# bcgsc/ntJoin

Hardware: AMD Instinct MI355X
Metric: Gbp/s minimizer-sketch+graph-build (k=32,w=1000) (higher is better)
Workload: dtype u64

## Files before the change

### ntjoin_amd/csrc/sketch.hip

```cpp
#include <algorithm>
#include <chrono>
#include <cmath>
#include <cstdlib>
#include <cstring>
#include <functional>
#include <type_traits>

#include "mxg_internal.h"
#include "nthash_dev.h"
#include "scan_kernels.h"
#include "sketch_bs.h"

namespace mxg {

enum Scratch {
    SC_CAND_H, SC_CAND_K, SC_CAND_C, SC_SEL, SC_BSUM, SC_CTRL, SC_ARENA, SC_STRIP_CNT, SC_STRIP_META,
    SC_GAPS, SC_WAVE_CNT, SC_ST_HASH, SC_ST_POS, SC_ST_REC, SC_ST_FWD, SC_G_HASH, SC_G_POS,
    SC_G_REC, SC_G_FWD, SC_V_RUNS, SC_V_STRIP0, SC_V_G0, SC_V_NK, SC_V_REC, SC_V_RUN0, SC_V_DROP, SC_CNT256, SC_WAVE_TOT,
    SC_GR_HASH, SC_GR_POS, SC_GR_REC, SC_GR_CNT, SC_GR_KEY, SC_GD_HASH, SC_GD_POS, SC_GD_REC,
    SC_CS_H, SC_CS_K, SC_CS_C,
    SC_GB_WORK,
    SC_COUNT
};
static_assert(SC_COUNT <= 40, "scratch pool too small");
// ... 2262 lines not shown
        if (rc != MXG_OK) return rc;
        return ev_end();
    }

    BsSelGeom sel_geom(const Assembly *a, const BatchGeom &g, double frac) const
    {
        return bs_select_geom(a->S_sparse, a->sel_H, h->cfg.w, frac, g.n_strips, (uint32_t)env_u64(h, "MXG_SEL_QCAP", 0), (uint32_t)env_u64(h, "MXG_SEL_RK", 0));
    }
    bool ctrl_cleared = false;
    int clear_sel_ctrl(const BsSelGeom &b)
    {
        int rc;
        if ((rc = flush_emit(nullptr)) != MXG_OK) return rc;
        const size_t ctrl_bytes = ((size_t)CTRL_WORDS + sup_words(b.n_slices) + 2 * 64 * 32) * 4;
        MXG_HIP(h, sc(SC_CTRL).ensure(ctrl_bytes));
        MXG_HIP(h, hipMemsetAsync(sc(SC_CTRL).p, 0, ctrl_bytes, st));
        ctrl_cleared = true;
        return MXG_OK;
    }
    int enqueue_sel(Assembly *a, const Tables &T, const BatchGeom &g, const BsSelGeom &b, uint32_t tau_hi, OutArrays &out,
                    uint32_t *ctrl_host, const ChainIO *io)
    {
        int rc;
        if ((rc = flush_emit(nullptr)) != MXG_OK) return rc;
        MXG_HIP(h, sc(SC_GAPS).ensure((size_t)GAP_CAP * 16));
        n_wave_sup = 0;
        const size_t ctrl_bytes = ((size_t)CTRL_WORDS + sup_words(b.n_slices) + 2 * 64 * 32) * 4;
        MXG_HIP(h, sc(SC_CTRL).ensure(ctrl_bytes));
        MXG_HIP(h, sc(SC_CNT256).ensure((size_t)b.n_slices * 4 + 64));
        const size_t n_ent = (size_t)b.n_slices * b.rk;
        MXG_HIP(h, sc(SC_CS_H).ensure(n_ent * 16));
        const size_t ovf_ent = (size_t)b.n_ovf * (b.ovf_cap + 2 * SEL_PAD);
        MXG_HIP(h, sc(SC_CAND_H).ensure(ovf_ent * 8));
        MXG_HIP(h, sc(SC_CAND_K).ensure(ovf_ent * 4));
        if (!ctrl_cleared) MXG_HIP(h, hipMemsetAsync(sc(SC_CTRL).p, 0, ctrl_bytes, st));
        ctrl_cleared = false;
        if ((rc = ev_begin(0, false, 2)) != MXG_OK) return rc;
        BsSelParams bp{};
        bp.bm = a->d_bs_out.as<uint32_t>() + 4;
        bp.packed = a->d_packed;
        bp.runx = a->d_runx.as<RunX>();
        bp.strip_run = T.d_strip_run;
        bp.ctg_drop = T.d_ctg_drop;
        bp.ptab = h->d_init_tab.as<uint4>() + 256;
        bp.n_strips_asm = (*T.strip0_sparse)[T.runs->size()];
        bp.strip_lo = g.strip_lo;
        bp.strip_hi = g.strip_hi;
        bp.S = a->S_sparse;
        bp.H = b.H;
        bp.T = b.T;
        bp.n_slices = b.n_slices;
        bp.w = h->cfg.w;
        bp.tau = (uint64_t)tau_hi << 32;
        bp.qcap = b.qcap;
        bp.ovf_h = sc(SC_CAND_H).as<uint64_t>();
        bp.ovf_e = sc(SC_CAND_K).as<uint32_t>();
        bp.ovf_cap = b.ovf_cap;
        bp.n_ovf = b.n_ovf;
        bp.ovf_next = sc(SC_CTRL).as<uint32_t>() + 12;
        bp.rk = b.rk;
        bp.cs = sc(SC_CS_H).as<uint4>();
        bp.cnt = sc(SC_CNT256).as<uint32_t>();
        bp.sup = sel_sup(0);
        bp.gaps = sc(SC_GAPS).as<uint4>();
        bp.gap_cap = GAP_CAP - SEL_IREQ_CAP;
        bp.ireq = sc(SC_GAPS).as<uint4>() + bp.gap_cap;
        bp.ireq_cap = SEL_IREQ_CAP - 8u;
        bp.gap_nmax = (io && io->dev_gaps && h->cfg.w <= ST_WMAX && !knob_set(h, "MXG_STRETCH_DENSE") && !knob_set(h, "MXG_GAP_WHOLE")) ? GAP_DEV_NMAX : 0u;
        bp.ctrl = sc(SC_CTRL).as<uint32_t>();
        bp.cand_spread = sel_sup(0) + sup_words(b.n_slices);
        bp.ablate = (uint32_t)env_u64(h, "MXG_SEL_ABLATE", 0);
        bp.inl_amax = knob_u64(h, "MXG_SEL_INLINE", 1) && b.n_slices < (1u << 24) ? bs_select_inline_amax(h->cfg.w) : 0u;
        if ((rc = launch_bs_select(h, bp, b, st)) != MXG_OK) return rc;
        const bool late = knob_u64(h, "MXG_STAGGER", 1) == 2;
        if (h->ev_sel_done[slot] && !late) MXG_HIP(h, hipEventRecord(h->ev_sel_done[slot], st));
        h->stat_sel_slices += b.n_slices;
        const bool dev = io && io->dev_gaps;
        if (timing && !fine) {
            if ((rc = ev_end()) != MXG_OK || (rc = ev_begin(0, false, 1)) != MXG_OK) return rc;
        }
        if ((rc = ev_next(3)) != MXG_OK) return rc;
        if (bp.inl_amax) {
            SelStretchParams sp{};
            sp.packed = bp.packed;
            sp.runs = T.d_runs;
            sp.ctg_run0 = T.d_ctg_run0;
            sp.ctg_drop = T.d_ctg_drop;
            sp.byte_tab = h->d_init_tab.as<uint4>();
            sp.tab = h->tab;
            sp.w = bp.w;
            sp.amax = bp.inl_amax;
            sp.rk = bp.rk;
            sp.cs = bp.cs;
            sp.cnt = bp.cnt;
            sp.sup = bp.sup;
            sp.ireq = bp.ireq;
            sp.ireq_cap = bp.ireq_cap;
            sp.ctrl = bp.ctrl;
            sp.tickets = bp.cand_spread + 64 * 32;
            sp.ablate = (uint32_t)env_u64(h, "MXG_SST_ABLATE", 0);
            sp.gaps = bp.gaps;
            sp.gap_cap = bp.gap_cap;
            sp.gap_nmax = bp.gap_nmax;
            if ((rc = launch_sel_stretch(h, sp, st)) != MXG_OK) return rc;
        }
        if (dev && (rc = enqueue_dev_gaps(a, T, ctrl_host)) != MXG_OK) return rc;
        if (defer_emit && io && !io->wait && !io->base_in && !io->base_out) {
            if ((rc = ev_end()) != MXG_OK) return rc;
            const Tables *Tp = &T;
            DevBuf *oh = out.hash, *op = out.pos, *orc = out.rec, *of = out.fwd;
            const uint64_t on = out.n;
            const ChainIO ioc = *io;
            const uint32_t rk = b.rk, gc = gcap, np = n_place;
            uint32_t *const no = n_out;
            const uint32_t *cs = bp.cand_spread;
            pending_emit = [=](hipEvent_t behind) -> int {
                int rc2;
                if (behind) MXG_HIP(h, hipStreamWaitEvent(st, behind, 0));
                if ((rc2 = ev_begin(0, false, fine ? 4 : 1)) != MXG_OK) return rc2;
                const uint32_t gc0 = gcap, np0 = n_place;
                uint32_t *const no0 = n_out;
                gcap = gc; n_place = np; n_out = no;
                rc2 = emit(a->d_packed, *Tp, (uint32_t)n_ent, *oh, *op, *orc, *of, on, true, ctrl_host, &ioc, rk, (uint32_t)n_ent, cs);
                gcap = gc0; n_place = np0; n_out = no0;
                if (rc2 != MXG_OK) return rc2;
                return ev_end();
            };
            return MXG_OK;
        }
        if ((rc = ev_next(4)) != MXG_OK) return rc;
        if (io && io->wait) MXG_HIP(h, hipStreamWaitEvent(st, io->wait, 0));
        rc = emit(a->d_packed, T, (uint32_t)n_ent, *out.hash, *out.pos, *out.rec, *out.fwd, out.n, true, ctrl_host, io, b.rk,
                  (uint32_t)n_ent, bp.cand_spread);
        if (rc != MXG_OK) return rc;
        if (h->ev_sel_done[slot] && late) MXG_HIP(h, hipEventRecord(h->ev_sel_done[slot], st));
        return ev_end();
    }
    std::function<int(hipEvent_t)> pending_emit;
    bool defer_emit = false;
    int flush_emit(hipEvent_t behind)
    {
        if (!pending_emit) return MXG_OK;
        auto f = std::move(pending_emit);
        pending_emit = nullptr;
        return f(behind);
    }

    int complete_batch(Assembly *a, const Tables &T, const BatchGeom &g, OutArrays &out, const uint32_t *ctrl, uint32_t n_cap)
    {
        const size_t c0 = g.c0, c1 = g.c1;
// ... 1359 lines not shown
```

### ntjoin_amd/csrc/sketch_bs.h

```cpp
#pragma once
#include "mxg_internal.h"

namespace mxg {

#ifndef MXG_BS_CHUNK_DEFINED
#define MXG_BS_CHUNK_DEFINED
constexpr uint32_t BS_CHUNK = 65536;
#endif

constexpr uint32_t SEL_PAD = 8;
constexpr uint32_t SEL_REQ = 8;
constexpr uint32_t SEL_GAP_DROP = 0x80000000u;
constexpr uint32_t SEL_MAX_H = 12;
constexpr uint32_t SEL_INL_R = 4;
constexpr uint32_t SEL_INL_PIECES = 6;
constexpr uint32_t SEL_INL_TMP = 128;
constexpr uint32_t SEL_IREQ_CAP = 1u << 18;

struct BsSelParams {
    const uint32_t *bm;
    const uint32_t *packed;
    const RunX *runx;
    const uint32_t *strip_run;
    const uint8_t *ctg_drop;
    const uint4 *ptab;
    uint32_t n_strips_asm;
    uint32_t strip_lo, strip_hi;
    uint32_t S, H, T;
    uint32_t n_slices;
    uint32_t w;
    uint64_t tau;
    uint32_t qcap;
    uint64_t *ovf_h;
    uint32_t *ovf_e;
    uint32_t ovf_cap, n_ovf;
    uint32_t *ovf_next;
    uint32_t rk;
    uint4 *cs;
    uint32_t *cnt, *sup;
    uint4 *gaps;
    uint32_t gap_cap;
    uint32_t gap_nmax;
    uint32_t *cand_spread;
    uint32_t *ctrl;
    uint32_t ablate;
    uint32_t inl_amax;
    uint4 *ireq;
    uint32_t ireq_cap;
};

struct SelStretchParams {
    const uint32_t *packed;
    const Run *runs;
    const uint32_t *ctg_run0;
    const uint8_t *ctg_drop;
    const uint4 *byte_tab;
    HashTab tab;
    uint32_t w, amax, rk;
    uint4 *cs;
    uint32_t *cnt, *sup;
    const uint4 *ireq;
    uint32_t ireq_cap;
    uint32_t *ctrl;
    uint32_t *tickets;
    uint4 *gaps;
    uint32_t gap_cap, gap_nmax;
    uint32_t ablate;
};
uint32_t bs_select_inline_amax(uint32_t w);
int launch_sel_stretch(mxg_handle *h, const SelStretchParams &p, hipStream_t st);

struct BsSelGeom {
    uint32_t H, T, n_slices, rk, qcap, waves, ovf_cap, n_ovf;
    size_t lds;
    bool ok;
};
uint32_t bs_select_halo(const Assembly *a, uint32_t S, uint32_t w);
BsSelGeom bs_select_geom(uint32_t S, uint32_t H, uint32_t w, double frac, uint32_t n_strips, uint32_t qcap_force, uint32_t rk_force = 0);
int launch_bs_select(mxg_handle *h, const BsSelParams &p, const BsSelGeom &g, hipStream_t st);

bool bs_possible(const mxg_handle *h, const Assembly *a);
int bs_prepare(mxg_handle *h, Assembly *a);
int bs_edges(mxg_handle *h, Assembly *a, hipStream_t st);
int bs_hash(mxg_handle *h, Assembly *a, uint32_t tau_hi, hipStream_t st);

}
```

### ntjoin_amd/csrc/sketch_bs.hip

```cpp
#include <algorithm>
#include <cmath>
#include <mutex>

#include "bs_kernels.h"
#include "nthash_dev.h"
#include "scan_kernels.h"
#include "sketch_bs.h"

namespace mxg {

namespace {

struct __attribute__((packed, aligned(4))) Words3 {
    uint32_t w0, w1, w2;
};
struct __attribute__((packed, aligned(4))) Words4 {
    uint32_t w0, w1, w2, w3;
};
template <int B>
__device__ __forceinline__ uint32_t byte_x16(const uint32_t x)
{
    uint32_t r;
#if defined(__HIP_DEVICE_COMPILE__)
    static_assert(B >= 0 && B < 4, "byte of a word");
// ... 48 lines not shown
__device__ __forceinline__ uint32_t sel_bits(const uint32_t w_lo, const uint32_t w_hi, const uint32_t sh, const uint32_t len, const uint32_t j)
{
    const uint32_t bits = __builtin_amdgcn_alignbit(w_hi, w_lo, sh);
    const uint32_t k0 = 32u * j;
    const uint32_t nvalid = len > k0 ? min(len - k0, 32u) : 0u;
    return bits & (nvalid >= 32u ? 0xFFFFFFFFu : ((1u << nvalid) - 1u));
}

struct StripRegs {
    uint64_t b;
    uint32_t len, cg, k0, nk;
};
__device__ __forceinline__ StripRegs strip_of(const BsSelParams &p, const bool in, const uint32_t sS, const uint32_t ri)
{
    StripRegs r;
    r.b = 0; r.len = 0; r.cg = 0xFFFFFFFFu; r.k0 = 0; r.nk = 0;
    if (in) {
        const RunX run = p.runx[ri];
        const uint32_t j0 = sS - run.strip0S;
        r.len = min(p.S, run.n_kmers - j0);
        r.b = run.base_off + j0;
        r.cg = run.contig;
        r.k0 = run.kidx0 + j0;
        r.nk = run.nk;
    }
    return r;
}
__device__ __forceinline__ StripRegs strip_from_run(const BsSelParams &p, const bool in, const uint32_t sS, const RunX &run)
{
    const uint32_t j0 = sS - run.strip0S;
    StripRegs r;
    r.len = in ? min(p.S, run.n_kmers - j0) : 0u;
    r.b = in ? run.base_off + j0 : 0ull;
    r.cg = in ? run.contig : 0xFFFFFFFFu;
    r.k0 = in ? run.kidx0 + j0 : 0u;
    r.nk = in ? run.nk : 0u;
    return r;
}
__device__ __forceinline__ StripRegs load_strip(const BsSelParams &p, const int64_t s64)
{
    const bool in = s64 >= 0 && s64 < (int64_t)p.n_strips_asm;
    const uint32_t s = in ? (uint32_t)s64 : 0u;
    return strip_of(p, in, s * p.S, in ? p.strip_run[s] : 0u);
}

__device__ __forceinline__ uint32_t wave_inclusive_dpp(uint32_t v)
{
    v += (uint32_t)__builtin_amdgcn_update_dpp(0, (int)v, 0x111, 0xf, 0xf, false);
    v += (uint32_t)__builtin_amdgcn_update_dpp(0, (int)v, 0x112, 0xf, 0xf, false);
    v += (uint32_t)__builtin_amdgcn_update_dpp(0, (int)v, 0x114, 0xf, 0xf, false);
    v += (uint32_t)__builtin_amdgcn_update_dpp(0, (int)v, 0x118, 0xf, 0xf, false);
    v += (uint32_t)__builtin_amdgcn_update_dpp(0, (int)v, 0x142, 0xa, 0xf, false);
    v += (uint32_t)__builtin_amdgcn_update_dpp(0, (int)v, 0x143, 0xc, 0xf, false);
    return v;
}

__device__ __forceinline__ const BsSelParams *sel_rare_params()
{
#if defined(__HIP_DEVICE_COMPILE__)
    const void *q = (const void *)__builtin_amdgcn_kernarg_segment_ptr();
    asm volatile("" : "+s"(q));
    return static_cast<const BsSelParams *>(q);
#else
    return nullptr;
#endif
}
__device__ __forceinline__ void push_gap(uint4 *gaps, uint32_t gap_cap, uint32_t *ctrl, uint32_t nmax, uint32_t w, uint32_t c, uint32_t lo,
                                         uint32_t hi, uint32_t hint)
{
    uint32_t s = lo, flag = 0u;
    for (;;) {
        const uint32_t e = nmax && hi - s >= nmax ? s + nmax - 1u : hi;
        const uint32_t idx = atomicAdd(&ctrl[1], 1u);
        if (idx < gap_cap) gaps[idx] = make_uint4(c, s, e, hint | flag);
        if (e == hi) break;
        s = e - w + 1u;
        flag = SEL_GAP_DROP;
    }
}
__device__ __forceinline__ void sel_push_gap(const BsSelParams &, uint32_t c, uint32_t lo, uint32_t hi, uint32_t hint)
{
    const BsSelParams *q = sel_rare_params();
    push_gap(q->gaps, q->gap_cap, q->ctrl, q->gap_nmax, q->w, c, lo, hi, hint);
}

__device__ __forceinline__ uint32_t stretch_end(const BsSelParams &p, const uint4 *ptab, const uint32_t lane, int64_t s_next, const uint32_t c,
                                                const uint32_t nk)
{
    const uint32_t nwords = (p.S + 31u) / 32u;
    for (;; s_next += 64) {
        const StripRegs r = load_strip(p, s_next + lane);
        const bool stop = r.cg != c;
        uint32_t kfound = 0xFFFFFFFFu;
        if (!stop) {
            const uint32_t *bw = p.bm + (r.b >> 5);
            const uint32_t sh = (uint32_t)r.b & 31u;
            uint32_t w0 = bw[0];
            for (uint32_t j = 0; j < nwords && kfound == 0xFFFFFFFFu; ++j) {
                const uint32_t w1 = bw[j + 1u];
                uint32_t bits = sel_bits(w0, w1, sh, r.len, j);
                w0 = w1;
                for (; bits; bits &= bits - 1u) {
                    const uint32_t ju = 32u * j + (uint32_t)__builtin_ctz(bits);
                    if (hash32_pos(p.packed, r.b + ju, ptab) < p.tau) {
                        kfound = r.k0 + ju;
                        break;
                    }
                }
            }
        }
        const uint64_t mf = __ballot(kfound != 0xFFFFFFFFu), ms = __ballot(stop);
        const uint64_t ev = mf | ms;
        if (ev) {
            const int first = __builtin_ctzll(ev);
            if ((mf >> first) & 1ull) return (uint32_t)__builtin_amdgcn_readlane((int)kfound, first) - 1u;
            return nk - 1u;
        }
    }
}

constexpr uint32_t SEL_SI = 6;

__host__ __device__ inline uint32_t sel_wave_lds(uint32_t qcap)
{
    return (qcap + 2u * SEL_PAD) * 12u + SEL_SI * 64u * 4u + SEL_REQ * 16u + SEL_REQ * 16u + 16u;
}

struct SelCtx {
    const uint4 *ptab;
    uint32_t *si;
    uint4 *req;
    uint32_t *misc;
    uint32_t lane, sl, own_end;
    bool has_drop;
    int64_t s_first;
    uint32_t nreal, own_lo, own_hi;
};

template <bool GLOB>
__device__ __forceinline__ void sel_sync()
{
    if (GLOB) __threadfence_block();
    else __builtin_amdgcn_wave_barrier();
}

template <int NB, bool GLOB>
__device__ __forceinline__ void sel_collect(const BsSelParams &p, SelCtx &c, uint64_t *lh, uint32_t *le, const uint32_t cap,
                                            const uint32_t (&bt)[NB], const uint32_t at0, const uint32_t tot)
{
    const uint32_t lane = c.lane, H = p.H;
    const uint32_t qn = min(tot, cap);
    {
        uint32_t at = at0;
#pragma unroll
        for (uint32_t j = 0; j < (uint32_t)NB; ++j) {
            uint32_t bits = bt[j];
            const uint32_t item0 = lane | ((32u * j) << 6);
            for (; bits; bits &= bits - 1u, ++at) le[at] = item0 + ((uint32_t)__builtin_ctz(bits) << 6);
        }
    }
    const uint32_t *s_blo = c.si, *s_bhi = c.si + 64, *s_f = c.si + 320;
    sel_sync<GLOB>();
    c.nreal = c.own_lo = c.own_hi = 0;
    if (p.ablate == 2) return;
    uint32_t nreal = 0, own_lo = 0, own_hi = 0;
    constexpr uint32_t NR = 4;
    for (uint32_t q0 = 0; q0 < qn; q0 += 64u * NR) {
        uint32_t item[NR];
        Words3 wv[NR];
        uint32_t shv[NR];
#pragma unroll
        for (uint32_t r = 0; r < NR; ++r) {
            const uint32_t q = q0 + 64u * r + lane;
            const bool act = q < qn;
            item[r] = act ? le[q] : 0u;
            const uint32_t l2 = item[r] & 63u;
            const uint64_t b = (((uint64_t)s_bhi[l2] << 32) | s_blo[l2]) + (item[r] >> 6);
            wv[r] = Words3{0u, 0u, 0u};
            if (act) wv[r] = *reinterpret_cast<const Words3 *>(p.packed + (b >> 4));
            shv[r] = ((uint32_t)b & 15u) * 2u;
        }
#pragma unroll
        for (uint32_t r = 0; r < NR; ++r) {
            if (q0 + 64u * r >= qn) break;
            const bool act = q0 + 64u * r + lane < qn;
            const uint32_t l2 = item[r] & 63u, ju = item[r] >> 6;
            const uint64_t h = act ? hash32_words(wv[r].w0, wv[r].w1, wv[r].w2, shv[r], c.ptab) : ~0ull;
            const bool real = act && h < p.tau;
            const uint64_t m = __ballot(real);
            const uint32_t rank = __builtin_amdgcn_mbcnt_hi((uint32_t)(m >> 32), __builtin_amdgcn_mbcnt_lo((uint32_t)m, 0u));
            if (real) {
                le[nreal + rank] = ((s_f[l2] + ju) << 6) | l2;
                lh[nreal + rank] = h;
            }
            own_lo += (uint32_t)__popcll(__ballot(real && l2 < H));
            own_hi += (uint32_t)__popcll(__ballot(real && l2 < c.own_end));
            nreal += (uint32_t)__popcll(m);
        }
    }
    if (lane < SEL_PAD) {
        le[-1 - (int)lane] = 0u;
        lh[-1 - (int)lane] = ~0ull;
        le[nreal + lane] = 0xFFFFFFFFu;
        lh[nreal + lane] = ~0ull;
    }
    sel_sync<GLOB>();
    c.nreal = nreal; c.own_lo = own_lo; c.own_hi = own_hi;
}

template <bool GLOB>
__device__ __forceinline__ void sel_decide(const BsSelParams &p, SelCtx &c, const uint64_t *lh, const uint32_t *le, const StripRegs &sr,
                                           const uint32_t f, bool &flag)
{
    const uint32_t lane = c.lane, sl = c.sl, H = p.H, w = p.w, wm1 = w - 1u, nreal = c.nreal;
    const bool has_drop = c.has_drop;
    const uint32_t lim = 64u * wm1 + 63u;
    const uint32_t *s_c = c.si + 128, *s_k0 = c.si + 192, *s_nk = c.si + 256, *s_f = c.si + 320;
    const uint32_t cov_c = (uint32_t)__builtin_amdgcn_readlane((int)sr.cg, 63);
    const uint32_t cov_kend = (uint32_t)__builtin_amdgcn_readlane((int)(sr.k0 + sr.len), 63);
    const uint32_t cov_nk = (uint32_t)__builtin_amdgcn_readlane((int)sr.nk, 63);
    const bool cov_open = cov_c != 0xFFFFFFFFu && cov_kend < cov_nk;
    auto push_req = [&](uint32_t cg, uint32_t lo, uint32_t hi) {
        const uint32_t q = atomicAdd(&c.misc[2], 1u);
        if (q < SEL_REQ) reinterpret_cast<uint4 *>(c.misc + 4)[q] = make_uint4(cg, lo, hi, 0u);
        else sel_push_gap(p, cg, lo, hi, sl * p.rk);
    };
    auto report = [&](uint32_t cg, uint32_t k_from, uint32_t nk, uint32_t nx) {
        bool same = false;
        uint32_t k2 = 0;
        if (nx < nreal) {
            const uint32_t e2 = le[nx], l2 = e2 & 63u;
            same = s_c[l2] == cg;
            k2 = s_k0[l2] + ((e2 >> 6) - s_f[l2]);
        }
        if (same) {
            if (k2 - k_from >= w) push_req(cg, k_from, k2 - 1u);
        } else if (nk - k_from >= w) {
            if (!(cov_open && cg == cov_c)) {
                push_req(cg, k_from, nk - 1u);
            } else {
                const uint32_t at = atomicAdd(&c.misc[0], 1u);
                if (at < SEL_REQ) c.req[at] = make_uint4(cg, k_from, nk, 0u);
            }
        }
    };
    uint32_t n_sel = 0;
    for (uint32_t i0 = c.own_lo; i0 < c.own_hi; i0 += 64u) {
        const bool live = i0 + lane < c.own_hi;
        const uint32_t i = live ? i0 + lane : i0;
        const uint32_t e = le[i], l1 = e & 63u;
        const uint64_t h = lh[i];
        const uint32_t kx = s_k0[l1] + ((e >> 6) - s_f[l1]), cg = s_c[l1], nk = s_nk[l1];
        const uint32_t e_lo = e - lim;
        uint32_t al = 0u;
        bool ldone = !live;
        for (uint32_t t = 1; !ldone; t += SEL_PAD) {
            uint32_t ae[SEL_PAD];
            uint64_t ah[SEL_PAD];
#pragma unroll
            for (uint32_t u = 0; u < SEL_PAD; ++u) {
// ... 23 lines not shown
            const uint32_t c0 = bh[0] <= h ? be[0] : n, c1 = bh[1] <= h ? be[1] : n, c2 = bh[2] <= h ? be[2] : n, c3 = bh[3] <= h ? be[3] : n;
            const uint32_t c4 = bh[4] <= h ? be[4] : n, c5 = bh[5] <= h ? be[5] : n, c6 = bh[6] <= h ? be[6] : n, c7 = bh[7] <= h ? be[7] : n;
            const uint32_t bl = min(min(min(c0, c1), c2), min(min(min(c3, c4), c5), min(c6, c7)));
            const bool blocked = bl <= e_hi;
            s = blocked ? false : s;
            rdone = blocked || be[SEL_PAD - 1] > e_hi;
        }
        if (has_drop && s && kx <= wm1 && L == kx && sel_rare_params()->ctg_drop[cg]) s = false;
        const uint64_t bm = __ballot(s);
        if (s) {
            const uint32_t dst = n_sel + __builtin_amdgcn_mbcnt_hi((uint32_t)(bm >> 32), __builtin_amdgcn_mbcnt_lo((uint32_t)bm, 0u));
            if (dst < p.rk) p.cs[(size_t)sl * p.rk + dst] = make_uint4((uint32_t)h, (uint32_t)(h >> 32), kx, cg);
        }
        n_sel += (uint32_t)__popcll(bm);
        if (live && le[i + 1u] - e >= 64u * (w + 1u)) report(cg, kx + 1u, nk, i + 1u);
    }
    if (lane >= H && lane < c.own_end && sr.len && sr.k0 == 0) {
        uint32_t lo = 0, hi = nreal;
        while (lo < hi) {
            const uint32_t mid = (lo + hi) >> 1;
            if ((le[mid] >> 6) < f) lo = mid + 1u; else hi = mid;
        }
        report(sr.cg, 0u, sr.nk, lo);
    }
    sel_sync<GLOB>();
    if (lane == 0) {
        if (n_sel > p.rk) flag = true;
        count_publish(p.cnt, p.sup, sl, min(n_sel, p.rk));
    }
    const uint32_t n_req = c.misc[0];
    if (n_req) {
        if (n_req > SEL_REQ) flag = true;
        for (uint32_t r = 0; r < min(n_req, SEL_REQ); ++r) {
            const uint4 rq = c.req[r];
            const uint32_t k_end = stretch_end(p, c.ptab, lane, c.s_first + 64, rq.x, rq.z);
            if (lane == 0 && k_end + 1u - rq.y >= w) push_req(rq.x, rq.y, k_end);
        }
        sel_sync<GLOB>();
        if (lane == 0) c.misc[0] = 0;
    }
    if (__builtin_expect(c.misc[2] != 0u, 0)) {
        const BsSelParams *pr = sel_rare_params();
        const uint32_t n_i = min(c.misc[2], SEL_REQ);
        const bool to_kernel = pr->inl_amax != 0u;
        uint32_t base = 0xFFFFFFFFu - SEL_REQ;
        if (to_kernel && lane == 0) base = atomicAdd(&pr->ctrl[15], n_i);
        base = (uint32_t)__builtin_amdgcn_readfirstlane((int)base);
        uint32_t ln = lane;
#if defined(__HIP_DEVICE_COMPILE__)
        asm volatile("" : "+v"(ln));
#endif
        if (ln < n_i) {
            const uint32_t *g = c.misc + 4u + 4u * ln;
            if (base + n_i <= pr->ireq_cap) pr->ireq[base + ln] = make_uint4(g[0], g[1], g[2], sl | (ln << 24) | (n_i << 27));
            else sel_push_gap(p, g[0], g[1], g[2], sl * pr->rk);
        }
        __builtin_amdgcn_wave_barrier();
        if (lane == 0) c.misc[2] = 0;
    }
}

}

template <int NWC, int NWX>
__global__ __launch_bounds__(1024) void k_bs_select(const BsSelParams p)
{
    static_assert(NWC % 4 == 0, "the strips' bitmap words are requested four at a time");
    static_assert(NWX < NWC, "one word more than the strip's bits is read (the bits are shifted into place)");
    constexpr int NB = NWX ? NWX : NWC - 1;
    extern __shared__ uint4 sel_lds[];
    uint4 *ptab = sel_lds;
    if ((uint32_t)(uintptr_t)sel_lds != 0u) __builtin_trap();
    for (uint32_t i = threadIdx.x; i < 2048u; i += blockDim.x) ptab[i] = p.ptab[i];
    const uint32_t lane = threadIdx.x & 63u, wib = threadIdx.x >> 6, nwv = blockDim.x >> 6;
    unsigned char *wb = reinterpret_cast<unsigned char *>(sel_lds + 2048) + (size_t)wib * sel_wave_lds(p.qcap);
    uint64_t *lh = reinterpret_cast<uint64_t *>(wb);
    uint32_t *le = reinterpret_cast<uint32_t *>(lh + p.qcap + 2u * SEL_PAD);
    SelCtx c;
    c.ptab = ptab;
    c.si = le + p.qcap + 2u * SEL_PAD;
    c.req = reinterpret_cast<uint4 *>(c.si + SEL_SI * 64u);
    c.misc = reinterpret_cast<uint32_t *>(c.req + SEL_REQ);
    c.lane = lane;
    c.has_drop = p.ctg_drop != nullptr;
    c.nreal = c.own_lo = c.own_hi = 0;
    uint32_t *blk_ticket = reinterpret_cast<uint32_t *>(reinterpret_cast<unsigned char *>(sel_lds + 2048) + (size_t)nwv * sel_wave_lds(p.qcap));
    if (threadIdx.x == 0) *blk_ticket = nwv;
    if (lane == 0) {
        c.misc[0] = 0;
        c.misc[2] = 0;
        c.misc[1] = 0xFFFFFFFFu;
    }
    __syncthreads();
    const uint32_t S = p.S, H = p.H, T = p.T, w = p.w;
    const uint32_t nwords = NWX ? (uint32_t)NWX : (S + 31u) / 32u;
    const uint32_t stride = gridDim.x * nwv, laneS = lane * S;
    uint32_t own_cands = 0;
    bool flag = false;
    auto slice_of = [&](uint32_t t) { return (t / nwv) * stride + blockIdx.x * nwv + (t % nwv); };
    uint32_t sl = slice_of(wib);
    const uint32_t sl_end = p.n_slices;
    auto first_strip = [&](uint32_t q) { return (int64_t)(p.strip_lo + q * T) - (int64_t)H; };
    StripRegs sr = sl < sl_end ? load_strip(p, first_strip(sl) + lane) : StripRegs{0, 0, 0xFFFFFFFFu, 0, 0};
    while (sl < sl_end) {
        uint32_t tk = 0;
        if (lane == 0) tk = atomicAdd(blk_ticket, 1u);
        const uint32_t sl_n = slice_of((uint32_t)__builtin_amdgcn_readfirstlane((int)tk));
        const uint32_t s_own0 = p.strip_lo + sl * T;
        c.sl = sl;
        c.s_first = first_strip(sl);
        c.own_end = H + min(T, p.strip_hi - s_own0);
        const uint32_t sn32 = p.strip_lo + sl_n * T - H + lane;
        const bool in_n = sl_n < sl_end && sn32 < p.n_strips_asm;
        const uint32_t s_n = in_n ? sn32 : 0u;
        const uint32_t ri_n = p.strip_run[s_n];
        const uint32_t sS_n = (sn32 - lane) * S + laneS;
        uint32_t wd[NWC];
        {
            const Words4 *bw = reinterpret_cast<const Words4 *>(p.bm + (sr.b >> 5));
#pragma unroll
            for (uint32_t u = 0; u < (uint32_t)NWC / 4u; ++u) {
                Words4 v{0u, 0u, 0u, 0u};
                if (sr.len && 4u * u <= nwords) v = bw[u];
                wd[4 * u] = v.w0; wd[4 * u + 1] = v.w1; wd[4 * u + 2] = v.w2; wd[4 * u + 3] = v.w3;
            }
        }
        const uint32_t len_p = (uint32_t)__builtin_amdgcn_update_dpp(0, (int)sr.len, 0x138, 0xf, 0xf, false);
        const uint32_t cg_p = (uint32_t)__builtin_amdgcn_update_dpp(-1, (int)sr.cg, 0x138, 0xf, 0xf, false);
        const uint32_t f = wave_inclusive_dpp(lane ? len_p + (sr.cg != cg_p ? w : 0u) : 2u * w);
        c.si[lane] = (uint32_t)sr.b;
        c.si[64u + lane] = (uint32_t)(sr.b >> 32);
        c.si[128u + lane] = sr.cg;
        c.si[192u + lane] = sr.k0;
        c.si[256u + lane] = sr.nk;
        c.si[320u + lane] = f;
        uint32_t bt[NB];
        uint32_t cnt = 0;
        {
            const uint32_t sh = (uint32_t)sr.b & 31u;
            const bool whole = (NWX || (S & 31u) == 0) && __ballot(sr.len != 0 && sr.len != S) == 0;
            if (whole) {
#pragma unroll
                for (uint32_t j = 0; j < (uint32_t)NB; ++j) bt[j] = j < nwords ? __builtin_amdgcn_alignbit(wd[j + 1], wd[j], sh) : 0u;
            } else {
#pragma unroll
                for (uint32_t j = 0; j < (uint32_t)NB; ++j) bt[j] = j < nwords ? sel_bits(wd[j], wd[j + 1], sh, sr.len, j) : 0u;
            }
#pragma unroll
            for (uint32_t j = 0; j < (uint32_t)NB; ++j) cnt += (uint32_t)__popc(bt[j]);
        }
        const uint32_t incl = wave_inclusive_dpp(cnt);
        const uint32_t tot = (uint32_t)__builtin_amdgcn_readlane((int)incl, 63);
        const RunX run_n = p.runx[ri_n];
        if (p.ablate == 1) {
            if (lane == 0) count_publish(p.cnt, p.sup, sl, 0u);
            own_cands += tot != 0;
        } else if (tot <= p.qcap) {
            sel_collect<NB, false>(p, c, lh + SEL_PAD, le + SEL_PAD, p.qcap, bt, incl - cnt, tot);
            if (p.ablate == 2 || p.ablate == 3) {
                if (lane == 0) count_publish(p.cnt, p.sup, sl, 0u);
                own_cands += 1u;
            } else {
                sel_decide<false>(p, c, lh + SEL_PAD, le + SEL_PAD, sr, f, flag);
            }
        } else {
            const BsSelParams *q = sel_rare_params();
            if (lane == 0 && c.misc[1] == 0xFFFFFFFFu) c.misc[1] = atomicAdd(q->ovf_next, 1u);
            __builtin_amdgcn_wave_barrier();
            const uint32_t region = c.misc[1];
            if (region < q->n_ovf) {
                const uint32_t ocap = q->ovf_cap;
                const size_t o = (size_t)region * (ocap + 2u * SEL_PAD) + SEL_PAD;
                sel_collect<NB, true>(p, c, q->ovf_h + o, q->ovf_e + o, ocap, bt, incl - cnt, tot);
                sel_decide<true>(p, c, q->ovf_h + o, q->ovf_e + o, sr, f, flag);
            } else {
                flag = true;
                c.own_lo = c.own_hi = 0;
                if (lane == 0) count_publish(p.cnt, p.sup, sl, 0u);
            }
        }
        own_cands += c.own_hi - c.own_lo;
        __builtin_amdgcn_wave_barrier();
        sr = strip_from_run(p, in_n, sS_n, run_n);
        sl = sl_n;
    }
    const uint32_t own_w = own_cands;
    if (lane == 0) {
        const BsSelParams *q = sel_rare_params();
        if (own_w) atomicAdd(&q->cand_spread[((blockIdx.x * nwv + wib) & 63u) * 32u], own_w);
        if (flag) q->ctrl[6] = q->ctrl[13] = 1;
    }
}

namespace {

struct InlBest {
    uint64_t h;
    uint32_t id;
};
template <int CTRL, int ROWS>
__device__ __forceinline__ InlBest inl_dpp(const InlBest v)
{
    InlBest o;
    const uint32_t lo = (uint32_t)__builtin_amdgcn_update_dpp(-1, (int)(uint32_t)v.h, CTRL, ROWS, 0xf, false);
    const uint32_t hi = (uint32_t)__builtin_amdgcn_update_dpp(-1, (int)(uint32_t)(v.h >> 32), CTRL, ROWS, 0xf, false);
    o.h = ((uint64_t)hi << 32) | lo;
    o.id = (uint32_t)__builtin_amdgcn_update_dpp(-1, (int)v.id, CTRL, ROWS, 0xf, false);
    return o;
}
template <bool OWN_LEFT>
__device__ __forceinline__ InlBest inl_scan(InlBest v)
{
#define MXG_INL_STEP(CTRL, ROWS)                                                   \
    {                                                                              \
        const InlBest g = inl_dpp<CTRL, ROWS>(v);                                  \
        const bool take = OWN_LEFT ? (g.id != 0xFFFFFFFFu && !(v.h < g.h)) : (g.h < v.h); \
        if (take) v = g;                                                           \
    }
    MXG_INL_STEP(0x111, 0xf)
    MXG_INL_STEP(0x112, 0xf)
    MXG_INL_STEP(0x114, 0xf)
    MXG_INL_STEP(0x118, 0xf)
    MXG_INL_STEP(0x142, 0xa)
    MXG_INL_STEP(0x143, 0xc)
#undef MXG_INL_STEP
    return v;
}
__device__ __forceinline__ InlBest inl_lane(const InlBest v, const int src_lane)
{
    InlBest o;
    o.h = __shfl(v.h, src_lane);
    o.id = __shfl(v.id, src_lane);
    return o;
}
// ... 120 lines not shown
        for (uint32_t r = 1; r < SEL_INL_R; ++r)
            if (r < R) last = ids[r];
        uint32_t prev = (uint32_t)__shfl((int)last, (int)lane - 1);
        if (lane == 0) prev = 0xFFFFFFFFu;
        uint32_t cnt = 0;
        bool em[SEL_INL_R];
#pragma unroll
        for (uint32_t r = 0; r < SEL_INL_R; ++r) {
            const uint32_t j = lane * R + r;
            em[r] = r < R && j <= a && ids[r] != prev && hs[r] != ~0ull && !(j == 0u && (lo != 0u || drop0));
            if (r < R && j <= a) prev = ids[r];
            cnt += em[r] ? 1u : 0u;
        }
        const uint32_t incl = wave_inclusive_dpp(cnt);
        const uint32_t tot = (uint32_t)__builtin_amdgcn_readlane((int)incl, 63);
        if (m + tot > cap_t) return 0xFFFFFFFFu;
        uint32_t at = m + incl - cnt;
#pragma unroll
        for (uint32_t r = 0; r < SEL_INL_R; ++r)
            if (em[r]) tmp[at++] = make_uint4((uint32_t)hs[r], (uint32_t)(hs[r] >> 32), k_from + lo + ids[r], cg);
        m += tot;
        __builtin_amdgcn_wave_barrier();
        if (lo + a >= a_tot) break;
        lo += a;
    }
    return m;
}

}

constexpr uint32_t SST_WAVES = 4;
__global__ __launch_bounds__(SST_WAVES * 64, 5) void k_sel_stretch(const SelStretchParams p)
{
    __shared__ uint4 byte_tab[256];
    __shared__ uint4 rtab[16];
    __shared__ uint64_t Xs[SST_WAVES][2 * 64 * SEL_INL_R];
    __shared__ uint4 tmps[SST_WAVES][SEL_INL_TMP];
    const uint32_t n_req = min(p.ctrl[15], p.ireq_cap);
    if (blockIdx.x * SST_WAVES >= n_req) return;
    for (uint32_t i = threadIdx.x; i < 256u; i += blockDim.x) byte_tab[i] = p.byte_tab[i];
    if (threadIdx.x < 16u) rtab[threadIdx.x] = p.tab.e[threadIdx.x];
    __syncthreads();
    const uint32_t lane = threadIdx.x & 63u, wv = threadIdx.x >> 6;
    uint64_t *X = Xs[wv];
    uint4 *tmp = tmps[wv];
    uint32_t *const ticket = p.tickets + ((blockIdx.x * SST_WAVES + wv) & 63u) * 32u;
    for (;;) {
        uint32_t r = 0;
        if (lane == 0) r = atomicAdd(ticket, 1u);
        r = (uint32_t)__builtin_amdgcn_readfirstlane((int)r) * 64u + ((blockIdx.x * SST_WAVES + wv) & 63u);
        if (r >= n_req) break;
        const uint4 mine = p.ireq[r + (lane & 7u)];
        const uint32_t w0 = (uint32_t)__builtin_amdgcn_readfirstlane((int)mine.w);
        if ((w0 >> 24) & 7u) continue;
        if (p.ablate & 8u) continue;
        const uint32_t n_i = min(w0 >> 27, SEL_REQ), sl = w0 & 0xFFFFFFu;
        const bool has = lane < n_i;
        const uint64_t my_key = has ? (((uint64_t)mine.x << 32) | mine.y) + 1ull : 0ull;
        uint4 *row = p.cs + (size_t)sl * p.rk;
        uint32_t n_cur = p.cnt[sl];
        uint64_t my_b = 0;
        bool my_ok = false;
        if (has) {
            uint32_t lo = p.ctg_run0[mine.x], hi = p.ctg_run0[mine.x + 1u];
            while (hi - lo > 1u) {
                const uint32_t mid = (lo + hi) >> 1;
                if (p.runs[mid].kidx0 <= mine.y) lo = mid; else hi = mid;
            }
            const Run run = p.runs[lo];
            my_ok = mine.z < run.kidx0 + run.n_kmers && mine.z - mine.y + 1u >= p.w && mine.z - mine.y + 1u - p.w <= p.amax * SEL_INL_PIECES;
            my_b = run.base_off + (mine.y - run.kidx0);
        }
        n_cur = (uint32_t)__builtin_amdgcn_readfirstlane((int)n_cur);
        uint4 e0 = make_uint4(0u, 0u, 0xFFFFFFFFu, 0xFFFFFFFFu), e1 = e0;
        if (lane < n_cur) e0 = row[lane];
        if (lane + 64u < n_cur) e1 = row[lane + 64u];
        const bool in_regs = n_cur <= 128u && n_i == 1u;
        uint32_t added = 0;
        uint64_t left = my_key;
        for (uint32_t it = 0; it < n_i; ++it) {
            uint64_t best = left;
#pragma unroll
            for (uint32_t d = 1; d < 8u; d <<= 1) {
                const uint64_t o = __shfl_xor(best, (int)d);
                best = o > best ? o : best;
            }
            best = __shfl(best, 0);
            const uint64_t holder = __ballot(left == best && best != 0ull);
            const int src = __builtin_ctzll(holder);
            if ((int)lane == src) left = 0ull;
            const uint32_t cg = (uint32_t)__shfl((int)mine.x, src), k_from = (uint32_t)__shfl((int)mine.y, src), k_to = (uint32_t)__shfl((int)mine.z, src);
            const uint64_t b_from = __shfl(my_b, src);
            const bool ok = __shfl((int)my_ok, src) != 0;
            const bool drop0 = k_from == 0u && p.ctg_drop && p.ctg_drop[cg];
            const uint64_t key = ((uint64_t)cg << 32) | k_from;
            uint32_t below = ((((uint64_t)e0.w << 32) | e0.z) < key ? 1u : 0u) + ((((uint64_t)e1.w << 32) | e1.z) < key ? 1u : 0u);
            for (uint32_t e = lane + 128u; e < n_cur - added; e += 64u) {
                const uint4 q = row[e];
                below += ((((uint64_t)q.w << 32) | q.z) < key) ? 1u : 0u;
            }
            uint32_t m = ok ? stretch_sketch(p, byte_tab, rtab, X, tmp, SEL_INL_TMP, cg, k_from, k_to, b_from, drop0) : 0xFFFFFFFFu;
            if (m != 0xFFFFFFFFu && n_cur + m > p.rk) m = 0xFFFFFFFFu;
            if (m == 0xFFFFFFFFu) {
                if (lane == 0) push_gap(p.gaps, p.gap_cap, p.ctrl, p.gap_nmax, p.w, cg, k_from, k_to, sl * p.rk);
                continue;
            }
            if (m == 0 || (p.ablate & 32u)) continue;
            const uint32_t at = wave_sum_u32(below);
            if (in_regs) {
// ... 204 lines not shown
```

Before: 2472.

## Prune dominated high-hash candidates before minimizer selection using low-hash coverage

Adds a lower hash threshold tau_lo (a fraction of tau, tunable through MXG_SEL_PRUNE) and, inside sel_collect, runs two wave-wide DPP max/min scans over the collected candidates. Candidates above tau_lo that sit between low-hash candidates spaced no more than w apart can never be window minimizers, so they are compacted away before sel_decide, and own counts are recomputed. This is meant to cut the work in the decide phase and in later stretch processing, at the cost of two extra passes over the candidate list and extra wave barriers. It also makes inline requests that overflow the request buffer write tombstones so the stretch kernel skips them, and adds a slice bounds check there.

```diff
diff --git a/ntjoin_amd/csrc/sketch.hip b/ntjoin_amd/csrc/sketch.hip
--- a/ntjoin_amd/csrc/sketch.hip
+++ b/ntjoin_amd/csrc/sketch.hip
@@ -2338,6 +2338,8 @@
         bp.n_slices = b.n_slices;
         bp.w = h->cfg.w;
         bp.tau = (uint64_t)tau_hi << 32;
+        const uint64_t prune = std::min<uint64_t>(env_u64(h, "MXG_SEL_PRUNE", 9), 23);
+        bp.tau_lo = tau_hi <= 0x80000000u ? (uint64_t)(((unsigned __int128)bp.tau * prune) / 24u) : 0ull;
         bp.qcap = b.qcap;
         bp.ovf_h = sc(SC_CAND_H).as<uint64_t>();
         bp.ovf_e = sc(SC_CAND_K).as<uint32_t>();
@@ -2352,6 +2354,7 @@
         bp.gap_cap = GAP_CAP - SEL_IREQ_CAP;
         bp.ireq = sc(SC_GAPS).as<uint4>() + bp.gap_cap;
         bp.ireq_cap = SEL_IREQ_CAP - 8u;
+        if (const uint64_t ic = env_u64(h, "MXG_SEL_IREQ_CAP", 0)) bp.ireq_cap = (uint32_t)std::min<uint64_t>(ic, bp.ireq_cap);
         bp.gap_nmax = (io && io->dev_gaps && h->cfg.w <= ST_WMAX && !knob_set(h, "MXG_STRETCH_DENSE") && !knob_set(h, "MXG_GAP_WHOLE")) ? GAP_DEV_NMAX : 0u;
         bp.ctrl = sc(SC_CTRL).as<uint32_t>();
         bp.cand_spread = sel_sup(0) + sup_words(b.n_slices);
@@ -2382,6 +2385,7 @@
             sp.sup = bp.sup;
             sp.ireq = bp.ireq;
             sp.ireq_cap = bp.ireq_cap;
+            sp.n_slices = bp.n_slices;
             sp.ctrl = bp.ctrl;
             sp.tickets = bp.cand_spread + 64 * 32;
             sp.ablate = (uint32_t)env_u64(h, "MXG_SST_ABLATE", 0);
diff --git a/ntjoin_amd/csrc/sketch_bs.h b/ntjoin_amd/csrc/sketch_bs.h
--- a/ntjoin_amd/csrc/sketch_bs.h
+++ b/ntjoin_amd/csrc/sketch_bs.h
@@ -16,6 +16,7 @@
 constexpr uint32_t SEL_INL_PIECES = 6;
 constexpr uint32_t SEL_INL_TMP = 128;
 constexpr uint32_t SEL_IREQ_CAP = 1u << 18;
+constexpr uint32_t SEL_IREQ_TOMB = 0xFFFFFFFFu;
 
 struct BsSelParams {
     const uint32_t *bm;
@@ -30,6 +31,7 @@
     uint32_t n_slices;
     uint32_t w;
     uint64_t tau;
+    uint64_t tau_lo;
     uint32_t qcap;
     uint64_t *ovf_h;
     uint32_t *ovf_e;
@@ -61,6 +63,7 @@
     uint32_t *cnt, *sup;
     const uint4 *ireq;
     uint32_t ireq_cap;
+    uint32_t n_slices;
     uint32_t *ctrl;
     uint32_t *tickets;
     uint4 *gaps;
diff --git a/ntjoin_amd/csrc/sketch_bs.hip b/ntjoin_amd/csrc/sketch_bs.hip
--- a/ntjoin_amd/csrc/sketch_bs.hip
+++ b/ntjoin_amd/csrc/sketch_bs.hip
@@ -124,6 +124,26 @@
     v += (uint32_t)__builtin_amdgcn_update_dpp(0, (int)v, 0x118, 0xf, 0xf, false);
     v += (uint32_t)__builtin_amdgcn_update_dpp(0, (int)v, 0x142, 0xa, 0xf, false);
     v += (uint32_t)__builtin_amdgcn_update_dpp(0, (int)v, 0x143, 0xc, 0xf, false);
+    return v;
+}
+__device__ __forceinline__ uint32_t wave_inclusive_max_dpp(uint32_t v)
+{
+    v = max(v, (uint32_t)__builtin_amdgcn_update_dpp(0, (int)v, 0x111, 0xf, 0xf, false));
+    v = max(v, (uint32_t)__builtin_amdgcn_update_dpp(0, (int)v, 0x112, 0xf, 0xf, false));
+    v = max(v, (uint32_t)__builtin_amdgcn_update_dpp(0, (int)v, 0x114, 0xf, 0xf, false));
+    v = max(v, (uint32_t)__builtin_amdgcn_update_dpp(0, (int)v, 0x118, 0xf, 0xf, false));
+    v = max(v, (uint32_t)__builtin_amdgcn_update_dpp(0, (int)v, 0x142, 0xa, 0xf, false));
+    v = max(v, (uint32_t)__builtin_amdgcn_update_dpp(0, (int)v, 0x143, 0xc, 0xf, false));
+    return v;
+}
+__device__ __forceinline__ uint32_t wave_inclusive_min_dpp(uint32_t v)
+{
+    v = min(v, (uint32_t)__builtin_amdgcn_update_dpp(-1, (int)v, 0x111, 0xf, 0xf, false));
+    v = min(v, (uint32_t)__builtin_amdgcn_update_dpp(-1, (int)v, 0x112, 0xf, 0xf, false));
+    v = min(v, (uint32_t)__builtin_amdgcn_update_dpp(-1, (int)v, 0x114, 0xf, 0xf, false));
+    v = min(v, (uint32_t)__builtin_amdgcn_update_dpp(-1, (int)v, 0x118, 0xf, 0xf, false));
+    v = min(v, (uint32_t)__builtin_amdgcn_update_dpp(-1, (int)v, 0x142, 0xa, 0xf, false));
+    v = min(v, (uint32_t)__builtin_amdgcn_update_dpp(-1, (int)v, 0x143, 0xc, 0xf, false));
     return v;
 }
 
@@ -207,6 +227,8 @@
     bool has_drop;
     int64_t s_first;
     uint32_t nreal, own_lo, own_hi;
+    uint32_t off;
+    uint32_t n_own;
 };
 
 template <bool GLOB>
@@ -215,6 +237,8 @@
     if (GLOB) __threadfence_block();
     else __builtin_amdgcn_wave_barrier();
 }
+
+constexpr uint64_t SEL_SHORT = 1ull << 63;
 
 template <int NB, bool GLOB>
 __device__ __forceinline__ void sel_collect(const BsSelParams &p, SelCtx &c, uint64_t *lh, uint32_t *le, const uint32_t cap,
@@ -233,8 +257,10 @@
     }
     const uint32_t *s_blo = c.si, *s_bhi = c.si + 64, *s_f = c.si + 320;
     sel_sync<GLOB>();
-    c.nreal = c.own_lo = c.own_hi = 0;
+    c.nreal = c.own_lo = c.own_hi = c.off = c.n_own = 0;
     if (p.ablate == 2) return;
+    const uint64_t tau_lo = p.tau_lo;
+    const uint32_t w = p.w;
     uint32_t nreal = 0, own_lo = 0, own_hi = 0;
     constexpr uint32_t NR = 4;
     for (uint32_t q0 = 0; q0 < qn; q0 += 64u * NR) {
@@ -270,6 +296,54 @@
             nreal += (uint32_t)__popcll(m);
         }
     }
+    c.n_own = own_hi - own_lo;
+    uint32_t off = 0;
+    if (tau_lo && p.ablate != 4) {
+        sel_sync<GLOB>();
+        uint32_t low_carry = 0;
+        for (uint32_t i0 = 0; i0 < nreal; i0 += 64u) {
+            const bool act = i0 + lane < nreal;
+            const uint32_t i = act ? i0 + lane : i0;
+            const uint32_t e = le[i];
+            const uint64_t h = lh[i];
+            const bool low = act && h < tau_lo;
+            const uint32_t incl = wave_inclusive_max_dpp(low ? e : 0u);
+            const uint32_t prev = max(low_carry, (uint32_t)__builtin_amdgcn_update_dpp(0, (int)incl, 0x138, 0xf, 0xf, false));
+            low_carry = max(low_carry, (uint32_t)__builtin_amdgcn_readlane((int)incl, 63));
+            if (low && prev && (e >> 6) - (prev >> 6) <= w) lh[i] = h | SEL_SHORT;
+        }
+        sel_sync<GLOB>();
+        const uint32_t own_end = c.own_end;
+        uint32_t top = nreal, n_lo = 0, n_hi = 0, key_carry = 0xFFFFFFFFu;
+        for (uint32_t hi = nreal; hi; hi = hi > 64u ? hi - 64u : 0u) {
+            const bool act = lane < hi;
+            const uint32_t i = act ? hi - 1u - lane : 0u;
+            const uint32_t e = le[i];
+            const uint64_t hs = lh[i], h = hs & ~SEL_SHORT;
+            const bool low = act && h < tau_lo;
+            const uint32_t incl = wave_inclusive_min_dpp(low ? (e << 1) | (uint32_t)(hs >> 63) : 0xFFFFFFFFu);
+            const uint32_t next = min(key_carry, (uint32_t)__builtin_amdgcn_update_dpp(-1, (int)incl, 0x138, 0xf, 0xf, false));
+            key_carry = min(key_carry, (uint32_t)__builtin_amdgcn_readlane((int)incl, 63));
+            const bool keep = act && (low || next == 0xFFFFFFFFu || !(next & 1u));
+            const uint64_t km = __ballot(keep);
+            const uint32_t rank = __builtin_amdgcn_mbcnt_hi((uint32_t)(km >> 32), __builtin_amdgcn_mbcnt_lo((uint32_t)km, 0u));
+            sel_sync<GLOB>();
+            if (keep) {
+                le[top - 1u - rank] = e;
+                lh[top - 1u - rank] = h;
+            }
+            const uint32_t l2 = e & 63u;
+            n_lo += (uint32_t)__popcll(__ballot(keep && l2 < H));
+            n_hi += (uint32_t)__popcll(__ballot(keep && l2 < own_end));
+            top -= (uint32_t)__popcll(km);
+        }
+        off = top;
+        nreal -= top;
+        own_lo = n_lo;
+        own_hi = n_hi;
+        le += off;
+        lh += off;
+    }
     if (lane < SEL_PAD) {
         le[-1 - (int)lane] = 0u;
         lh[-1 - (int)lane] = ~0ull;
@@ -277,7 +351,7 @@
         lh[nreal + lane] = ~0ull;
     }
     sel_sync<GLOB>();
-    c.nreal = nreal; c.own_lo = own_lo; c.own_hi = own_hi;
+    c.nreal = nreal; c.own_lo = own_lo; c.own_hi = own_hi; c.off = off;
 }
 
 template <bool GLOB>
@@ -407,8 +481,10 @@
 #endif
         if (ln < n_i) {
             const uint32_t *g = c.misc + 4u + 4u * ln;
-            if (base + n_i <= pr->ireq_cap) pr->ireq[base + ln] = make_uint4(g[0], g[1], g[2], sl | (ln << 24) | (n_i << 27));
-            else sel_push_gap(p, g[0], g[1], g[2], sl * pr->rk);
+            const bool fits = base + n_i <= pr->ireq_cap;
+            const uint4 rq = make_uint4(g[0], g[1], g[2], sl | (ln << 24) | (n_i << 27));
+            if (fits || base + ln < pr->ireq_cap) pr->ireq[base + ln] = fits ? rq : make_uint4(0u, 0u, 0u, SEL_IREQ_TOMB);
+            if (!fits) sel_push_gap(p, rq.x, rq.y, rq.z, sl * pr->rk);
         }
         __builtin_amdgcn_wave_barrier();
         if (lane == 0) c.misc[2] = 0;
@@ -438,7 +514,7 @@
     c.misc = reinterpret_cast<uint32_t *>(c.req + SEL_REQ);
     c.lane = lane;
     c.has_drop = p.ctg_drop != nullptr;
-    c.nreal = c.own_lo = c.own_hi = 0;
+    c.nreal = c.own_lo = c.own_hi = c.off = c.n_own = 0;
     uint32_t *blk_ticket = reinterpret_cast<uint32_t *>(reinterpret_cast<unsigned char *>(sel_lds + 2048) + (size_t)nwv * sel_wave_lds(p.qcap));
     if (threadIdx.x == 0) *blk_ticket = nwv;
     if (lane == 0) {
@@ -512,11 +588,11 @@
             own_cands += tot != 0;
         } else if (tot <= p.qcap) {
             sel_collect<NB, false>(p, c, lh + SEL_PAD, le + SEL_PAD, p.qcap, bt, incl - cnt, tot);
-            if (p.ablate == 2 || p.ablate == 3) {
+            if (p.ablate >= 2 && p.ablate <= 4) {
                 if (lane == 0) count_publish(p.cnt, p.sup, sl, 0u);
                 own_cands += 1u;
             } else {
-                sel_decide<false>(p, c, lh + SEL_PAD, le + SEL_PAD, sr, f, flag);
+                sel_decide<false>(p, c, lh + SEL_PAD + c.off, le + SEL_PAD + c.off, sr, f, flag);
             }
         } else {
             const BsSelParams *q = sel_rare_params();
@@ -527,14 +603,14 @@
                 const uint32_t ocap = q->ovf_cap;
                 const size_t o = (size_t)region * (ocap + 2u * SEL_PAD) + SEL_PAD;
                 sel_collect<NB, true>(p, c, q->ovf_h + o, q->ovf_e + o, ocap, bt, incl - cnt, tot);
-                sel_decide<true>(p, c, q->ovf_h + o, q->ovf_e + o, sr, f, flag);
+                sel_decide<true>(p, c, q->ovf_h + o + c.off, q->ovf_e + o + c.off, sr, f, flag);
             } else {
                 flag = true;
-                c.own_lo = c.own_hi = 0;
+                c.own_lo = c.own_hi = c.n_own = 0;
                 if (lane == 0) count_publish(p.cnt, p.sup, sl, 0u);
             }
         }
-        own_cands += c.own_hi - c.own_lo;
+        own_cands += c.n_own;
         __builtin_amdgcn_wave_barrier();
         sr = strip_from_run(p, in_n, sS_n, run_n);
         sl = sl_n;
@@ -761,9 +837,10 @@
         if (r >= n_req) break;
         const uint4 mine = p.ireq[r + (lane & 7u)];
         const uint32_t w0 = (uint32_t)__builtin_amdgcn_readfirstlane((int)mine.w);
-        if ((w0 >> 24) & 7u) continue;
+        if (w0 == SEL_IREQ_TOMB || ((w0 >> 24) & 7u)) continue;
         if (p.ablate & 8u) continue;
         const uint32_t n_i = min(w0 >> 27, SEL_REQ), sl = w0 & 0xFFFFFFu;
+        if (sl >= p.n_slices) continue;
         const bool has = lane < n_i;
         const uint64_t my_key = has ? (((uint64_t)mine.x << 32) | mine.y) + 1ull : 0ull;
         uint4 *row = p.cs + (size_t)sl * p.rk;
```

Result: no change. 2476, median of 5 (+0.1%).
